# cscott/compressjs

Measured on AMD Instinct MI355X. Metric: bzip2 -9 compress MB/s on enwik8-shaped input, higher is better.
Workload: dtype u8; 1 GPU; synthetic enwik8-shaped text with phrase reuse calibrated to enwik8's bzip2 -9 ratio (compressjs_amd.synth.enwik_like, seed 2025), 100000000 bytes per GPU, bzip2 -9, 899981-byte blocks; BASELINE.json configs[2]; input_bytes=100000000, compressed_bytes=29488912, blocks_in_flight=128

## Files before the change

compressjs_amd/csrc/devutil.h:

```cpp
#pragma once
#include "cjs_common.h"

extern "C" __device__ int cjs_writelane(int val, int lane, int old) __asm("llvm.amdgcn.writelane.i32");

__device__ __forceinline__ u64 bitset1_b64(u64 m, u32 b) {
#if defined(__AMDGCN__)
    asm("s_bitset1_b64 %0, %1" : "+s"(m) : "s"(b));
    return m;
#else
    return m | (1ull << (b & 63u));
#endif
}

__device__ __forceinline__ u64 bitset0_b64(u64 m, u32 b) {
#if defined(__AMDGCN__)
    asm("s_bitset0_b64 %0, %1" : "+s"(m) : "s"(b));
    return m;
#else
    return m & ~(1ull << (b & 63u));
#endif
}

__device__ __forceinline__ u32 be_sel(u32 sh) {
#if defined(__AMDGCN__)
// ... 20 lines not shown
#if defined(__AMDGCN__)
    asm volatile("s_waitcnt lgkmcnt(0)\n\ts_barrier" ::: "memory");
#else
    __syncthreads();
#endif
}

__device__ __forceinline__ u64 match_any(u32 d, int nbits, bool valid) {
    u64 m = __ballot(valid);
    for (int i = 0; i < nbits; i++) {
        const bool bit = (d >> i) & 1u;
        const u64 b = __ballot(bit);
        m &= bit ? b : ~b;
    }
    return m;
}

__device__ __forceinline__ u32 block_excl_scan_256(u32 v, u32* sh) {
    const u32 tid = threadIdx.x;
    if (tid < 256) sh[tid] = v;
    __syncthreads();
    for (u32 off = 1; off < 256; off <<= 1) {
        u32 t = 0;
        if (tid < 256 && tid >= off) t = sh[tid - off];
        __syncthreads();
        if (tid < 256) sh[tid] += t;
        __syncthreads();
    }
    const u32 incl = tid < 256 ? sh[tid] : 0;
    __syncthreads();
    return incl - v;
}


__device__ __forceinline__ u32 wave_incl_scan_u32(u32 v) {
    const u32 lane = threadIdx.x & 63u;
    for (u32 off = 1; off < 64; off <<= 1) {
        const u32 u = __shfl_up(v, off);
        if (lane >= off) v += u;
    }
    return v;
}

__device__ __forceinline__ u32 wave_incl_scan_dpp(u32 v) {
    v += (u32)__builtin_amdgcn_update_dpp(0, (int)v, 0x111, 0xf, 0xf, true);
    v += (u32)__builtin_amdgcn_update_dpp(0, (int)v, 0x112, 0xf, 0xf, true);
    v += (u32)__builtin_amdgcn_update_dpp(0, (int)v, 0x114, 0xf, 0xf, true);
    v += (u32)__builtin_amdgcn_update_dpp(0, (int)v, 0x118, 0xf, 0xf, true);
    v += (u32)__builtin_amdgcn_update_dpp(0, (int)v, 0x142, 0xa, 0xf, false);
    v += (u32)__builtin_amdgcn_update_dpp(0, (int)v, 0x143, 0xc, 0xf, false);
    return v;
}
__device__ __forceinline__ u32 wave_sum_dpp(u32 v) { return (u32)__builtin_amdgcn_readlane((int)wave_incl_scan_dpp(v), 63); }

__device__ __forceinline__ u32 block_excl_scan_1024(u32 v, u32* sh, u32* total) {
    const u32 tid = threadIdx.x, w = tid >> 6, lane = tid & 63u;
    const u32 nw = (blockDim.x + 63u) >> 6;
    const u32 incl = wave_incl_scan_u32(v);
    if (lane == 63u) sh[w] = incl;
    __syncthreads();
    if (w == 0) {
        const u32 t = lane < nw ? sh[lane] : 0u;
        const u32 ti = wave_incl_scan_u32(t);
        if (lane < nw) sh[lane] = ti - t;
        if (lane == 63u) sh[17] = ti;
    }
    __syncthreads();
    const u32 r = sh[w] + incl - v;
    *total = sh[17];
    __syncthreads();
    return r;
}


__device__ __forceinline__ bool xcd_block_tile(u32 nb, u32& b, u32& t) {
    const u32 T = gridDim.x;
    const u32 L = blockIdx.x + T * blockIdx.y;
    const u32 xcd = L & 7u, r = L >> 3;
    t = r % T;
    b = xcd + 8u * (r / T);
    return b < nb;
}
```

compressjs_amd/csrc/k0_plan.h:

```cpp
#pragma once
#include "pipeline.h"
#include "devutil.h"

#define K0_TILE 4096
#define K0_NONE 0ull

__device__ __forceinline__ u32 k0_g(u64 k) {
    const u64 q = k / 255u;
    const u32 r = (u32)(k - q * 255u);
    return (u32)(5u * q) + (r < 4u ? r : 5u);
}
__device__ __forceinline__ u32 k0_c(u64 k) {
    const u32 sub = (u32)(k % 255u);
    return sub < 3u ? 1u : (sub == 3u ? 2u : 0u);
}

__device__ __forceinline__ void load16(const K0Buf& K, u64 j0, u8* b) {
    if (j0 + 16u <= K.in_len && ((((uintptr_t)K.in) + j0) & 15u) == 0) {
        const uint4 v = *(const uint4*)(K.in + j0);
        const u32 w[4] = {v.x, v.y, v.z, v.w};
#pragma unroll
        for (int k = 0; k < 16; k++) b[k] = (u8)(w[k >> 2] >> (8 * (k & 3)));
    } else {
#pragma unroll
        for (int k = 0; k < 16; k++) b[k] = j0 + k < K.in_len ? K.in[j0 + k] : 0;
    }
}

__device__ __forceinline__ u64 tile_runstarts(const K0Buf& K, u64 t, u64 rs_in, u8* b, u64* sh, u32& hm) {
    const u32 tid = threadIdx.x;
    const u64 j0 = t * K0_TILE + tid * 16u;
    u8 prev = 0;
    if (j0 > 0 && j0 - 1 < K.in_len) prev = K.in[j0 - 1];
    load16(K, j0, b);
    const u32 nv = j0 >= K.in_len ? 0u : (K.in_len - j0 < 16u ? (u32)(K.in_len - j0) : 16u);
    u32 heads = (j0 == 0 || b[0] != prev) ? 1u : 0u;
#pragma unroll
    for (int k = 1; k < 16; k++) heads |= b[k] != b[k - 1] ? 1u << k : 0u;
    heads &= (1u << nv) - 1u;
    hm = heads;
    u32 v = heads ? tid * 16u + 32u - (u32)__clz((int)heads) : 0u;
    const u32 lane = tid & 63u, w = tid >> 6;
    u32* sh32 = (u32*)sh;
    for (u32 off = 1; off < 64; off <<= 1) {
        const u32 u = (u32)__shfl_up((int)v, off);
        if (lane >= off && u > v) v = u;
    }
    if (lane == 63u) sh32[w] = v;
    __syncthreads();
    u32 before = (u32)__shfl_up((int)v, 1u);
    if (lane == 0) before = 0;
    for (u32 ww = 0; ww < w; ww++) if (sh32[ww] > before) before = sh32[ww];
    __syncthreads();
    return before ? t * K0_TILE + before - 1u : rs_in;
}
__device__ __forceinline__ u64 tile_runstarts(const K0Buf& K, u64 t, u64 rs_in, u8* b, u64* sh) {
    u32 hm;
    return tile_runstarts(K, t, rs_in, b, sh, hm);
}
__device__ __forceinline__ u32 k0_mod255(u64 d) { return (d >> 32) ? (u32)(d % 255u) : (u32)d % 255u; }

static __device__ u64 k0_evalC(const K0Buf& K, u64 i, u64* sh, u32* sh32) {
    if (i >= K.in_len) return K.tileC[K.ntiles];
// ... 126 lines not shown
```

compressjs_amd/csrc/k0_rle1.hip:

```cpp
#include "pipeline.h"
#include "crc_dev.h"
#include "devutil.h"
#include "k0_plan.h"

#define K0_TPW 4u
__global__ __launch_bounds__(256) void k0_tile_last(K0Buf K) {
    const u32 tid = threadIdx.x, lane = tid & 63u, w = tid >> 6;
    __shared__ u64 wl[K0_TPW][4];
    u8 b[K0_TPW][16];
    u8 prev[K0_TPW];
#pragma unroll
    for (u32 q = 0; q < K0_TPW; q++) {
        const u64 j0 = ((u64)blockIdx.x * K0_TPW + q) * K0_TILE + tid * 16u;
        prev[q] = 0;
        if (j0 < K.in_len) {
            load16(K, j0, b[q]);
            if (j0) prev[q] = K.in[j0 - 1];
        }
    }
#pragma unroll
    for (u32 q = 0; q < K0_TPW; q++) {
        const u64 j0 = ((u64)blockIdx.x * K0_TPW + q) * K0_TILE + tid * 16u;
        u64 mine = K0_NONE;
        if (j0 < K.in_len) {
#pragma unroll
            for (int k = 0; k < 16; k++) {
                const u64 j = j0 + k;
                if (j < K.in_len && (j == 0 || b[q][k] != (k ? b[q][k - 1] : prev[q]))) mine = j + 1;
            }
        }
        const u64 has = __ballot(mine != K0_NONE);
        const u64 top = __shfl(mine, has ? 63 - __clzll((long long)has) : 0);
        if (lane == 0) wl[q][w] = has ? top : K0_NONE;
    }
    __syncthreads();
    if (tid < K0_TPW) {
        const u64 t = (u64)blockIdx.x * K0_TPW + tid;
        if (t < K.ntiles) {
            u64 last = K0_NONE;
            for (u32 ww = 0; ww < 4u; ww++) if (wl[tid][ww] != K0_NONE) last = wl[tid][ww];
            K.tileA[t] = last;
            K.tileB[t] = last;
        }
    }
}

template <bool MAX>
__device__ __forceinline__ u64 scan_op(u64 a, u64 b) { return MAX ? (a > b ? a : b) : a + b; }

template <bool MAX>
__global__ __launch_bounds__(256) void k0_scan_local(u64* data, u64* chunkTot, u64 n) {
    __shared__ u64 sh[256];
    const u64 c0 = (u64)blockIdx.x * 1024u;
    const u32 tid = threadIdx.x;
    u64 v[4], run = 0;
    for (int k = 0; k < 4; k++) {
        const u64 i = c0 + tid * 4u + k;
        v[k] = i < n ? data[i] : 0;
    }
    u64 tot = 0;
    for (int k = 0; k < 4; k++) tot = scan_op<MAX>(tot, v[k]);
    sh[tid] = tot;
    __syncthreads();
    for (u32 off = 1; off < 256; off <<= 1) {
        u64 tv = 0;
        if (tid >= off) tv = sh[tid - off];
        __syncthreads();
        if (tid >= off) sh[tid] = scan_op<MAX>(sh[tid], tv);
        __syncthreads();
    }
    run = tid ? sh[tid - 1] : 0;
    for (int k = 0; k < 4; k++) {
        const u64 i = c0 + tid * 4u + k;
        if (i < n) data[i] = run;
        run = scan_op<MAX>(run, v[k]);
    }
    if (tid == 255) chunkTot[blockIdx.x] = sh[255];
}

template <bool MAX>
__global__ __launch_bounds__(1024) void k0_scan_chunks(u64* chunkTot, u64 nchunks, u64* total, u64* reset) {
    __shared__ u64 sh[1024];
    __shared__ u64 carry;
    const u32 tid = threadIdx.x;
    if (tid == 0) carry = 0;
    __syncthreads();
    for (u64 c0 = 0; c0 < nchunks; c0 += 1024) {
        const u64 i = c0 + tid;
        const u64 v = i < nchunks ? chunkTot[i] : 0;
        sh[tid] = v;
        __syncthreads();
        for (u32 off = 1; off < 1024; off <<= 1) {
            u64 tv = 0;
            if (tid >= off) tv = sh[tid - off];
            __syncthreads();
            if (tid >= off) sh[tid] = scan_op<MAX>(sh[tid], tv);
            __syncthreads();
        }
        const u64 ex = scan_op<MAX>(carry, tid ? sh[tid - 1] : 0);
        if (i < nchunks) chunkTot[i] = ex;
        __syncthreads();
        if (tid == 1023) carry = scan_op<MAX>(carry, sh[1023]);
        __syncthreads();
    }
    if (tid == 0 && total) *total = carry;
    if (tid == 0 && reset) *reset = ~0ull;
}

template <bool MAX>
__global__ __launch_bounds__(256) void k0_scan_apply(u64* data, const u64* chunkTot, u64 n) {
    const u64 c0 = (u64)blockIdx.x * 1024u;
    const u64 base = chunkTot[blockIdx.x];
    for (int k = 0; k < 4; k++) {
        const u64 i = c0 + (u64)k * 256u + threadIdx.x;
        if (i < n) data[i] = scan_op<MAX>(base, data[i]);
    }
}

__global__ __launch_bounds__(256) void k0_tile_cost(K0Buf K) {
    const u64 t = blockIdx.x;
    __shared__ u64 sh[256];
    __shared__ u32 tot;
    if (threadIdx.x == 0) tot = 0;
    u8 b[16];
    const u64 rsin_raw = K.tileA[t];
    const u64 rs_in = rsin_raw != K0_NONE ? rsin_raw - 1 : 0;
    u32 hm;
    const u64 rs = tile_runstarts(K, t, rs_in, b, sh, hm);
    const u64 j0 = t * K0_TILE + threadIdx.x * 16u;
    const u32 nv = j0 >= K.in_len ? 0u : (K.in_len - j0 < 16u ? (u32)(K.in_len - j0) : 16u);
    u32 c = 0, sub = 0;
    if (nv) {
        sub = (hm & 1u) ? 0u : k0_mod255(j0 - rs);
        c = sub < 3u ? 1u : (sub == 3u ? 2u : 0u);
#pragma unroll
        for (u32 k = 1; k < 16; k++) {
            sub = ((hm >> k) & 1u) ? 0u : (sub == 254u ? 0u : sub + 1u);
            c += k < nv ? (sub < 3u ? 1u : (sub == 3u ? 2u : 0u)) : 0u;
        }
    }
    const u32 wsum = wave_incl_scan_dpp(c);
    if ((threadIdx.x & 63u) == 63u) atomicAdd(&tot, wsum);
    __syncthreads();
    if (threadIdx.x == 0) K.tileC[t] = tot;
}

__global__ __launch_bounds__(256) void k0_chain_spec(K0Buf K, u32 cap) {
    __shared__ u64 sh[256];
    __shared__ u32 sh32[4];
    const u64 total = K.tileC[K.ntiles];
    const u64 nfull = total / cap;
    const u64 j = (u64)blockIdx.x + 1;
    if (j > nfull) return;
    u64 ce = 0;
    const u64 e = k0_searchC(K, j * (u64)cap, 0, sh, sh32, &ce);
    if (threadIdx.x == 0) {
        bool bad = e > K.in_len || ce != j * (u64)cap;
        if (!bad && e < K.in_len && e > 0 && K.in[e - 1] == K.in[e]) {
            const u8 c = K.in[e];
            u32 len = 2;
            for (u64 q = e + 1; q < K.in_len && len < 4 && K.in[q] == c; q++) len++;
            for (u64 q = e - 1; q > 0 && len < 4 && K.in[q - 1] == c; q--) len++;
            bad = len >= 4;
        }
        K.specEnd[j] = e;
        K.specC[j] = ce;
        if (bad) atomicMin((unsigned long long*)K.specBad, (unsigned long long)j);
    }
}

__global__ __launch_bounds__(256) void k0_chain(K0Buf K, u32 cap) {
    __shared__ u64 sh[256];
    __shared__ u32 sh32[4];
    const u64 total = K.tileC[K.ntiles];
    const u64 nfull = total / cap;
    u64 kb0 = *K.specBad < nfull ? *K.specBad : nfull;
    if (kb0 > K.maxBlocks) kb0 = K.maxBlocks;
    for (u64 k = threadIdx.x; k < kb0; k += 256u) {
        const u64 s0 = k ? K.specEnd[k] : 0;
        K.blkStart[k] = s0;
        K.blkEnd[k] = K.specEnd[k + 1];
        K.blkN[k] = cap;
        K.blkAdj[k] = k * (u64)cap;
        K.blkRe[k] = s0;
    }
    u64 s = kb0 ? K.specEnd[kb0] : 0, cnext = kb0 ? K.specC[kb0] : 0;
    bool have_cnext = true;
    u32 kb = (u32)kb0;
    while (s < K.in_len && kb < K.maxBlocks) {
        const bool cut = s > 0 && K.in[s - 1] == K.in[s];
        u64 e = s, adj = 0, re = s;
        u32 n = 0;
        bool done = false;
        u64 pre = 0, cbase = 0;
        if (cut) {
            re = k0_run_end(K, s, sh);
            const u64 L = re - s;
// ... 142 lines not shown
__global__ __launch_bounds__(1024) void k0_crc(K0Buf K, Pipe P, u32 first_block) {
    const u32 b = blockIdx.y, kb = first_block + b;
    if (kb >= *K.nBlocks) return;
    const u64 s = K.blkStart[kb], e = K.blkEnd[kb];
    const u32 parts = gridDim.x;
    __shared__ u32 tab[CRC_TAB_WORDS];
    __shared__ u32 pw[40];
    __shared__ u32 acc;
    const u64 part = (((e - s + parts - 1u) / parts) + 15u) & ~(u64)15;
    const u64 ps = s + blockIdx.x * part < e ? s + blockIdx.x * part : e;
    const u64 pe = ps + part < e ? ps + part : e;
    if (ps >= pe) return;
    const u32 c = crc_range_raw(K.in, ps, pe, e, tab, pw, &acc);
    if (threadIdx.x == 0) atomicXor(&P.crc[b], c);
}

size_t k0_bytes(u64 in_len, u32 cap) {
    const u64 ntiles = (in_len + K0_TILE - 1) / K0_TILE;
    const u64 nchunks = (ntiles + 1 + 1023) / 1024;
    const u64 maxBlocks = in_len / (cap / 2 + 1) + 2;
    size_t tot = 0;
    tot += 3 * (((ntiles + 2) * 8 + 255) & ~(size_t)255);
    tot += ((nchunks + 1) * 8 + 255) & ~(size_t)255;
    tot += 6 * (((maxBlocks + 2) * 8 + 255) & ~(size_t)255) + ((maxBlocks * 4 + 255) & ~(size_t)255) + 512;
    return tot;
}

void k0_carve(K0Buf& K, const u8* d_in, u64 in_len, u32 cap, void* ws) {
    K.in = d_in;
    K.in_len = in_len;
    K.ntiles = (in_len + K0_TILE - 1) / K0_TILE;
    K.nchunks = (K.ntiles + 1 + 1023) / 1024;
    K.maxBlocks = (u32)(in_len / (cap / 2 + 1) + 2);
    char* p = (char*)ws;
    const size_t ta = ((K.ntiles + 2) * 8 + 255) & ~(size_t)255;
    K.tileA = (u64*)p; p += ta;
    K.tileB = (u64*)p; p += ta;
    K.tileC = (u64*)p; p += ta;
    K.chunk = (u64*)p; p += ((K.nchunks + 1) * 8 + 255) & ~(size_t)255;
    const size_t bb = ((size_t)K.maxBlocks * 8 + 255) & ~(size_t)255;
    K.blkStart = (u64*)p; p += bb;
    K.blkEnd = (u64*)p; p += bb;
    K.blkAdj = (u64*)p; p += bb;
    K.blkRe = (u64*)p; p += bb;
    K.blkN = (u32*)p; p += ((size_t)K.maxBlocks * 4 + 255) & ~(size_t)255;
    const size_t sb = (((size_t)K.maxBlocks + 2) * 8 + 255) & ~(size_t)255;
    K.specEnd = (u64*)p; p += sb;
    K.specC = (u64*)p; p += sb;
    K.nBlocks = (u32*)p; p += 256;
    K.specBad = (u64*)p;
}

int k0_scans(K0Buf K, hipStream_t stream) {
    const u32 nt = (u32)K.ntiles, nc = (u32)K.nchunks;
    hipLaunchKernelGGL(k0_tile_last, dim3((nt + K0_TPW - 1u) / K0_TPW), dim3(256), 0, stream, K);
    hipLaunchKernelGGL(k0_scan_local<true>, dim3(nc), dim3(256), 0, stream, K.tileA, K.chunk, K.ntiles);
    hipLaunchKernelGGL(k0_scan_chunks<true>, dim3(1), dim3(1024), 0, stream, K.chunk, K.nchunks, (u64*)nullptr, (u64*)nullptr);
    hipLaunchKernelGGL(k0_scan_apply<true>, dim3(nc), dim3(256), 0, stream, K.tileA, (const u64*)K.chunk, K.ntiles);
    hipLaunchKernelGGL(k0_tile_cost, dim3(nt), dim3(256), 0, stream, K);
    hipLaunchKernelGGL(k0_scan_local<false>, dim3(nc), dim3(256), 0, stream, K.tileC, K.chunk, K.ntiles);
    hipLaunchKernelGGL(k0_scan_chunks<false>, dim3(1), dim3(1024), 0, stream, K.chunk, K.nchunks, K.tileC + K.ntiles, K.specBad);
    hipLaunchKernelGGL(k0_scan_apply<false>, dim3(nc), dim3(256), 0, stream, K.tileC, (const u64*)K.chunk, K.ntiles);
    HIP_CHECK_RET(hipGetLastError());
    return CJS_OK;
}

int k0_prepass(K0Buf K, u32 cap, hipStream_t stream) {
    if (K.in_len == 0) {
        HIP_CHECK_RET(hipMemsetAsync(K.nBlocks, 0, 4, stream));
        return CJS_OK;
    }
    const int rc = k0_scans(K, stream);
    if (rc) return rc;
    const u32 nspec = (u32)(K.in_len * 5 / 4 / cap + 2 < K.maxBlocks ? K.in_len * 5 / 4 / cap + 2 : K.maxBlocks);
    hipLaunchKernelGGL(k0_chain_spec, dim3(nspec), dim3(256), 0, stream, K, cap);
    hipLaunchKernelGGL(k0_chain, dim3(1), dim3(256), 0, stream, K, cap);
    HIP_CHECK_RET(hipGetLastError());
    return CJS_OK;
}

__global__ __launch_bounds__(256) void k0_phase_spec(K0Buf K, u32 cap, u64 t0) {
    __shared__ u64 sh[256];
    __shared__ u32 sh32[4];
    const u64 total = K.tileC[K.ntiles];
    const u64 m = blockIdx.x;
    const u64 t = t0 + m * (u64)cap;
    if (t > total) { if (threadIdx.x == 0) { K.specEnd[m] = K.in_len + 1; K.specC[m] = 0; } return; }
    u64 ce = 0, e = 0;
    if (t) e = k0_searchC(K, t, 0, sh, sh32, &ce);
    if (threadIdx.x == 0) {
        bool bad = e > K.in_len || ce != t;
        if (!bad && e < K.in_len && e > 0 && K.in[e - 1] == K.in[e]) {
            const u8 c = K.in[e];
            u32 len = 2;
            for (u64 q = e + 1; q < K.in_len && len < 4 && K.in[q] == c; q++) len++;
            for (u64 q = e - 1; q > 0 && len < 4 && K.in[q - 1] == c; q--) len++;
            bad = len >= 4;
        }
        K.specEnd[m] = e;
        K.specC[m] = ce;
        if (bad) atomicMin((unsigned long long*)K.specBad, (unsigned long long)m);
    }
}

__global__ __launch_bounds__(256) void k0_phase_chain(K0Buf K, u32 cap, u64 t0, u64 own_len, u32 last, u32 nbound) {
    __shared__ u64 sh[256];
    __shared__ u32 sh32[4];
    __shared__ u32 nb, fail, stop;
    const u32 tid = threadIdx.x;
    if (tid == 0) { nb = 0; fail = 0; stop = nbound; }
    __syncthreads();
    const u64 total = K.tileC[K.ntiles];
    const u64 badraw = *K.specBad;
    const u32 bad = badraw < (u64)nbound ? (u32)badraw : nbound;
    for (u32 m = tid; m < nbound; m += 256u) {
// ... 113 lines not shown
```

compressjs_amd/csrc/k5_pack.hip:

```cpp
#include "pipeline.h"

__device__ __forceinline__ u32 bswap32(u32 v) {
    return (v >> 24) | ((v >> 8) & 0xFF00u) | ((v << 8) & 0xFF0000u) | (v << 24);
}

__device__ __forceinline__ void put_bits_lds(u32* words, u32 pos, u32 nbits, u32 value) {
    if (nbits == 0) return;
    const u32 wi = pos >> 5, sh = pos & 31u;
    const u64 v = ((u64)value << (64u - nbits)) >> sh;
    atomicOr(&words[wi], (u32)(v >> 32));
    const u32 lo = (u32)v;
    if (lo) atomicOr(&words[wi + 1], lo);
}

__device__ __forceinline__ u32 mtf6_index(u32 list, u32 s) {
    u32 j = 0;
    while (((list >> (4u * j)) & 15u) != s) j++;
    return j;
}
__device__ __forceinline__ u32 mtf6_front(u32 list, u32 j, u32 s) {
    const u32 lowmask = (1u << (4u * j)) - 1u;
    const u32 keep = list & ~((lowmask << 4) | 15u);
    return keep | ((list & lowmask) << 4) | s;
}

#define K5_MAX_SEL 18432
__global__ __launch_bounds__(256) void k5_header(Pipe P) {
    const u32 b = blockIdx.x;
    const u32 n = P.nlen[b];
    const u32 tid = threadIdx.x;
    if (n == 0) { if (tid == 0) P.hbits[b] = 0; return; }
    __shared__ u32 hw[K5_HDR_WORDS];
    __shared__ u32 sh[256];
    __shared__ int lastT[6][256];
    __shared__ u32 s_cursor;
    for (u32 i = tid; i < K5_HDR_WORDS; i += 256) hw[i] = 0;
    __syncthreads();
    const u32 alpha = P.alpha[b], G = P.ngroups[b], nSel = P.nsel[b];
    const int S = (int)alpha + 2;
    __shared__ __attribute__((aligned(16))) u8 sel[K5_MAX_SEL];
    {
        const u8* gsel = P.sel + (size_t)b * P.selPitch;
        const u32 nw4 = ((nSel < K5_MAX_SEL ? nSel : K5_MAX_SEL) + 3u) >> 2;
        for (u32 i = tid; i < nw4; i += 256) ((u32*)sel)[i] = ((const u32*)gsel)[i];
    }
    if (tid == 0) {
        put_bits_lds(hw, 0, 24, 0x314159u);
        put_bits_lds(hw, 24, 24, 0x265359u);
        put_bits_lds(hw, 48, 32, P.crc[b]);
        put_bits_lds(hw, 80, 1, 0);
        put_bits_lds(hw, 81, 24, P.pidx[b]);
        const u32* used8 = P.used + (size_t)b * 8;
        u32 cur = 105, map = 0;
        for (int i = 0; i < 16; i++) {
            const u32 r = (used8[i >> 1] >> ((i & 1) * 16)) & 0xFFFFu;
            if (r) map |= 1u << (15 - i);
        }
        put_bits_lds(hw, cur, 16, map);
        cur += 16;
        for (int i = 0; i < 16; i++) {
            const u32 r = (used8[i >> 1] >> ((i & 1) * 16)) & 0xFFFFu;
            if (r) {
                u32 rev = 0;
                for (int j = 0; j < 16; j++) if (r & (1u << j)) rev |= 1u << (15 - j);
                put_bits_lds(hw, cur, 16, rev);
                cur += 16;
            }
        }
        put_bits_lds(hw, cur, 3, G);
        put_bits_lds(hw, cur + 3, 15, nSel);
        s_cursor = cur + 18;
    }
    __syncthreads();
    u32 cursor = s_cursor;
    if (alpha >= G) {
        const u32 chunk = (nSel + 255u) / 256u;
        const u32 lo = tid * chunk < nSel ? tid * chunk : nSel;
        const u32 hi = lo + chunk < nSel ? lo + chunk : nSel;
        int lastp[6];
#pragma unroll
        for (int t = 0; t < 6; t++) lastp[t] = K5_NONE;
        for (u32 i = lo; i < hi; i++) {
            const u32 s = sel[i];
#pragma unroll
            for (int t = 0; t < 6; t++) if (s == (u32)t) lastp[t] = (int)i;
        }
#pragma unroll
        for (int t = 0; t < 6; t++) lastT[t][tid] = lastp[t];
        __syncthreads();
        if (tid < 6) {
            int cur = -1 - (int)tid;
            for (int k = 0; k < 256; k++) {
                const int v = lastT[tid][k];
                lastT[tid][k] = cur;
                cur = cur > v ? cur : v;
            }
        }
        __syncthreads();
        u32 list = 0;
        {
            int Ls[6];
#pragma unroll
            for (int t = 0; t < 6; t++) Ls[t] = lastT[t][tid];
#pragma unroll
            for (int t = 0; t < 6; t++) {
                u32 r = 0;
#pragma unroll
                for (int u = 0; u < 6; u++) r += (Ls[u] > Ls[t]) ? 1u : 0u;
                list |= (u32)t << (4u * r);
            }
        }
        const u32 list0 = list;
        u32 bits = 0;
        for (u32 i = lo; i < hi; i++) {
            const u32 s = sel[i];
            const u32 j = mtf6_index(list, s);
            list = mtf6_front(list, j, s);
            bits += j + 1u;
        }
        u32 off = cursor + block_excl_scan_256(bits, sh);
        list = list0;
        for (u32 i = lo; i < hi; i++) {
            const u32 s = sel[i];
            const u32 j = mtf6_index(list, s);
            list = mtf6_front(list, j, s);
            put_bits_lds(hw, off, j + 1u, ((1u << j) - 1u) << 1);
            off += j + 1u;
        }
        __syncthreads();
        if (tid == 255) s_cursor = off;
        __syncthreads();
        cursor = s_cursor;
    } else {
        if (tid == 0) {
            int M[6];
            const int mlen = (int)alpha;
            for (int i = 0; i < mlen; i++) M[i] = i;
            u32 off = cursor;
            for (u32 i = 0; i < nSel; i++) {
                const int s = sel[i];
                int j;
                for (j = 0; j < (int)G; j++) if (j < mlen && M[j] == s) break;
                const int src = j < mlen ? M[j] : 0;
                for (int k = j; k > 0; k--) if (k < mlen) M[k] = M[k - 1];
                if (mlen > 0) M[0] = src;
                put_bits_lds(hw, off, (u32)j + 1u, ((1u << j) - 1u) << 1);
                off += (u32)j + 1u;
            }
            s_cursor = off;
        }
        __syncthreads();
        cursor = s_cursor;
    }
    for (u32 t = 0; t < G; t++) {
        const u8* lens = P.lens + ((size_t)b * CJS_MAX_GROUPS + t) * CJS_LEN_PITCH;
        if (tid == 0) put_bits_lds(hw, cursor, 5, lens[0]);
        u32 nb0 = 0, nb1 = 0;
        const int i0 = 2 * (int)tid, i1 = i0 + 1;
        int l0 = 0, lp0 = 0, l1 = 0;
        if (i0 < S) { l0 = lens[i0]; lp0 = i0 ? lens[i0 - 1] : l0; nb0 = 2u * (u32)(l0 > lp0 ? l0 - lp0 : lp0 - l0) + 1u; }
        if (i1 < S) { l1 = lens[i1]; nb1 = 2u * (u32)(l1 > l0 ? l1 - l0 : l0 - l1) + 1u; }
        u32 off = cursor + 5u + block_excl_scan_256(nb0 + nb1, sh);
        if (i0 < S) {
            const u32 val = lp0 < l0 ? 2u : 3u;
            for (u32 d = 0; d + 1u < nb0; d += 2u) put_bits_lds(hw, off + d, 2, val);
            off += nb0;
        }
        if (i1 < S) {
            const u32 val = l0 < l1 ? 2u : 3u;
            for (u32 d = 0; d + 1u < nb1; d += 2u) put_bits_lds(hw, off + d, 2, val);
            off += nb1;
        }
        __syncthreads();
        if (tid == 255) s_cursor = off;
        __syncthreads();
        cursor = s_cursor;
    }
    const u32 nw = (cursor + 31u) >> 5;
    u32* out = P.hdr + (size_t)b * K5_HDR_WORDS;
    for (u32 i = tid; i < nw; i += 256) out[i] = hw[i];
    if (tid == 0) P.hbits[b] = cursor;
}

__global__ __launch_bounds__(256) void k5_tilescan(Pipe P) {
    const BatchGeom g = P.g;
    const u32 b = blockIdx.x, tid = threadIdx.x;
    __shared__ u32 sh[256];
    __shared__ u32 carry;
    const u32 nSel = P.nlen[b] ? P.nsel[b] : 0u;
    if (tid == 0) carry = P.nlen[b] ? P.hbits[b] : 0u;
    __syncthreads();
    const u16* cost = P.selCost + (size_t)b * P.selPitch;
    u32* cnt = P.tileBits + (size_t)b * K5_TILES(g);
    for (u32 t0 = 0; t0 < K5_TILES(g); t0 += 256) {
        const u32 t = t0 + tid;
        u32 v = 0;
        const u32 g0 = t * K5_TGROUPS;
        if (g0 + K5_TGROUPS <= nSel) {
            const uint4* c4 = (const uint4*)(cost + g0);
#pragma unroll
            for (u32 k = 0; k < K5_TGROUPS / 8u; k++) {
                const uint4 q = c4[k];
                v += (q.x & 0xFFFFu) + (q.x >> 16) + (q.y & 0xFFFFu) + (q.y >> 16) + (q.z & 0xFFFFu) + (q.z >> 16) + (q.w & 0xFFFFu) + (q.w >> 16);
            }
        } else for (u32 gi = g0; gi < nSel; gi++) v += cost[gi];
        const u32 ex = block_excl_scan_256(v, sh);
        const u32 base = carry;
        if (t < K5_TILES(g)) cnt[t] = base + ex;
        __syncthreads();
        if (tid == 255) carry = base + ex + v;
        __syncthreads();
    }
    if (tid == 0) P.bitlen[b] = carry;
}

__global__ __launch_bounds__(64) void k5_blockscan(Pipe P) {
    if (threadIdx.x != 0) return;
    u64 bits = P.ss->bits;
    u32 crc = P.ss->crc;
    for (u32 b = 0; b < P.g.nb; b++) {
        P.bitoff[b] = bits;
        if (P.nlen[b]) {
            bits += P.bitlen[b];
            crc = ((crc << 1) | (crc >> 31)) ^ P.crc[b];
        }
    }
    if (((bits + 80u + 7u) >> 3) + 8u > P.outCapBytes) P.ss->overflow = 1;
    P.ss->bits = bits;
    P.ss->crc = crc;
    if (P.snap) *P.snap = bits;
}

#define K5_STAGE_WORDS ((K5_TILE * 20u + 62u) / 32u + 2u)
__device__ __forceinline__ void or_word(u32* out, u64 wi, u32 word) {
    if (word) atomicOr(&out[wi], bswap32(word));
}

__global__ __launch_bounds__(256) void k5_pack(Pipe P) {
    const BatchGeom g = P.g;
    const u32 b = blockIdx.y, t = blockIdx.x;
    if (P.nlen[b] == 0 || P.ss->overflow) return;
    const u32 pos = P.pos[b];
    const u32 t0 = t * K5_TILE;
    const u32 tid = threadIdx.x;
    const u64 boff = P.bitoff[b];
    if (t == 0) {
        const u32 hb = P.hbits[b];
        const u32 nw = (hb + 31u) >> 5;
        const u32* hdr = P.hdr + (size_t)b * K5_HDR_WORDS;
        const u32 s = (u32)(boff & 31u);
        const u64 w0 = boff >> 5;
        for (u32 k = tid; k <= nw; k += 256) {
            const u32 cur = k < nw ? hdr[k] : 0u;
            const u32 prev = k > 0 ? hdr[k - 1] : 0u;
            const u32 v = s ? ((prev << (32u - s)) | (cur >> s)) : cur;
            or_word(P.out, w0 + k, v);
        }
    }
    if (t0 >= pos) return;
    __shared__ u32 codes[CJS_MAX_GROUPS][CJS_LEN_PITCH];
    __shared__ u32 sh[256];
    __shared__ u32 stage[K5_STAGE_WORDS];
    __shared__ u32 s_tot;
    const u32 G = P.ngroups[b];
// ... 48 lines not shown
            }
        }
        if (nacc) atomicOr(&stage[wi], (u32)(acc << (32u - nacc)));
    }
    __syncthreads();
    for (u32 j = tid; j < nw; j += 256) {
        const u32 v = stage[j];
        if (j == 0u || j + 1u == nw) or_word(P.out, w0 + j, v);
        else P.out[w0 + j] = bswap32(v);
    }
}

__global__ void k5_begin(Pipe P, int level) {
    if (threadIdx.x == 0 && blockIdx.x == 0) {
        if (level > 0) P.out[0] = bswap32(0x425A6800u | (u32)('0' + level));
        P.ss->bits = level > 0 ? 32 : 0;
        P.ss->crc = 0;
        P.ss->overflow = 0;
    }
}
__global__ void k5_end(Pipe P) {
    if (threadIdx.x != 0 || blockIdx.x != 0 || P.ss->overflow) return;
    const u64 pos = P.ss->bits;
    const u32 parts[3] = {0x177245u, 0x385090u, P.ss->crc};
    const u32 nb[3] = {24, 24, 32};
    u64 p = pos;
    for (int k = 0; k < 3; k++) {
        const u32 sh = (u32)(p & 31u);
        const u64 v = ((u64)parts[k] << (64u - nb[k])) >> sh;
        or_word(P.out, p >> 5, (u32)(v >> 32));
        or_word(P.out, (p >> 5) + 1, (u32)v);
        p += nb[k];
    }
    P.ss->bits = p;
}

int k5_stream_begin(Pipe P, int level, hipStream_t stream, bool zero) {
    if (zero) HIP_CHECK_RET(hipMemsetAsync(P.out, 0, P.outCapBytes, stream));
    hipLaunchKernelGGL(k5_begin, dim3(1), dim3(64), 0, stream, P, level);
    HIP_CHECK_RET(hipGetLastError());
    return CJS_OK;
}

int k5_stream_end(Pipe P, hipStream_t stream) {
    hipLaunchKernelGGL(k5_end, dim3(1), dim3(64), 0, stream, P);
    HIP_CHECK_RET(hipGetLastError());
    return CJS_OK;
}

int k5_run(Pipe P, u32 max_n, hipStream_t stream, hipEvent_t after, hipEvent_t done, hipEvent_t crc_ready, const K5Docs* docs, u32 first_block) {
    const BatchGeom g = P.g;
    const u32 tiles = (max_n + 1 + K5_TILE - 1) / K5_TILE;
    if (crc_ready) HIP_CHECK_RET(hipStreamWaitEvent(stream, crc_ready, 0));
    hipLaunchKernelGGL(k5_header, dim3(g.nb), dim3(256), 0, stream, P);
    hipLaunchKernelGGL(k5_tilescan, dim3(g.nb), dim3(256), 0, stream, P);
    if (after) HIP_CHECK_RET(hipStreamWaitEvent(stream, after, 0));
    if (docs) {
        const int rc = k5_docscan_run(P, *docs, first_block, stream);
        if (rc) return rc;
    } else hipLaunchKernelGGL(k5_blockscan, dim3(1), dim3(64), 0, stream, P);
    if (done) HIP_CHECK_RET(hipEventRecord(done, stream));
    hipLaunchKernelGGL(k5_pack, dim3(tiles, g.nb), dim3(256), 0, stream, P);
    HIP_CHECK_RET(hipGetLastError());
    return CJS_OK;
}

__global__ __launch_bounds__(256) void k5_shift_bits(const u8* in, u64 nbytes, u32 s, u8* out) {
    const u64 i = (u64)blockIdx.x * 256u + threadIdx.x;
    if (i > nbytes) return;
    const u32 cur = i < nbytes ? in[i] : 0u;
    const u32 prev = i ? in[i - 1] : 0u;
    out[i] = (u8)((cur >> s) | (prev << (8u - s)));
}
int k5_shift_bits_run(const u8* d_in, u64 nbytes, u32 s, u8* d_out, hipStream_t stream) {
    hipLaunchKernelGGL(k5_shift_bits, dim3((u32)((nbytes + 256) / 256)), dim3(256), 0, stream, d_in, nbytes, s & 7u, d_out);
    HIP_CHECK_RET(hipGetLastError());
    return CJS_OK;
}
```

Baseline: 15710 MB/s.

## Fuse RLE1 tile scans into two kernels and merge header with tilescan

Replaces the eight-kernel RLE1 planning sequence (tile-last, three-pass max scan, tile-cost, three-pass sum scan) with a tile summary kernel that computes last run start, leading-run length and in-tile cost in one pass, plus a single 1024-thread kernel that does both scans and fixes up the cost of the leading run algebraically. The bzip2 header kernel grows to 1024 threads, uses DPP wave scans instead of serial LDS scans, stores MTF positions so the selector MTF pass runs once, writes all code-length deltas in one scan, and absorbs the tilescan kernel. The aim is to cut launch count, serial single-thread loops and repeated input reads. The cost is a single-block scan over all tiles and more complex carry and boundary logic.

```diff
diff --git a/compressjs_amd/csrc/devutil.h b/compressjs_amd/csrc/devutil.h
--- a/compressjs_amd/csrc/devutil.h
+++ b/compressjs_amd/csrc/devutil.h
@@ -96,6 +96,18 @@
     return v;
 }
 __device__ __forceinline__ u32 wave_sum_dpp(u32 v) { return (u32)__builtin_amdgcn_readlane((int)wave_incl_scan_dpp(v), 63); }
+template <bool MAX>
+__device__ __forceinline__ u32 wave_incl_scan_dpp_op(u32 v) {
+#define CJS_DPP_STEP(ctrl, rows, bc) { const u32 u = (u32)__builtin_amdgcn_update_dpp(0, (int)v, ctrl, rows, 0xf, bc); v = MAX ? (u > v ? u : v) : v + u; }
+    CJS_DPP_STEP(0x111, 0xf, true)
+    CJS_DPP_STEP(0x112, 0xf, true)
+    CJS_DPP_STEP(0x114, 0xf, true)
+    CJS_DPP_STEP(0x118, 0xf, true)
+    CJS_DPP_STEP(0x142, 0xa, false)
+    CJS_DPP_STEP(0x143, 0xc, false)
+#undef CJS_DPP_STEP
+    return v;
+}
 
 __device__ __forceinline__ u32 block_excl_scan_1024(u32 v, u32* sh, u32* total) {
     const u32 tid = threadIdx.x, w = tid >> 6, lane = tid & 63u;
diff --git a/compressjs_amd/csrc/k0_plan.h b/compressjs_amd/csrc/k0_plan.h
--- a/compressjs_amd/csrc/k0_plan.h
+++ b/compressjs_amd/csrc/k0_plan.h
@@ -9,6 +9,10 @@
     const u64 q = k / 255u;
     const u32 r = (u32)(k - q * 255u);
     return (u32)(5u * q) + (r < 4u ? r : 5u);
+}
+__device__ __forceinline__ u32 k0_g32(u32 k) {
+    const u32 q = k / 255u, r = k - q * 255u;
+    return 5u * q + (r < 4u ? r : 5u);
 }
 __device__ __forceinline__ u32 k0_c(u64 k) {
     const u32 sub = (u32)(k % 255u);
diff --git a/compressjs_amd/csrc/k0_rle1.hip b/compressjs_amd/csrc/k0_rle1.hip
--- a/compressjs_amd/csrc/k0_rle1.hip
+++ b/compressjs_amd/csrc/k0_rle1.hip
@@ -4,9 +4,11 @@
 #include "k0_plan.h"
 
 #define K0_TPW 4u
-__global__ __launch_bounds__(256) void k0_tile_last(K0Buf K) {
+__device__ __forceinline__ u32 k0_cost_of(u32 sub) { return sub < 3u ? 1u : (sub == 3u ? 2u : 0u); }
+
+__global__ __launch_bounds__(256) void k0_tile_summary(K0Buf K) {
     const u32 tid = threadIdx.x, lane = tid & 63u, w = tid >> 6;
-    __shared__ u64 wl[K0_TPW][4];
+    __shared__ u32 wlast[K0_TPW][4], wfirst[K0_TPW][4], wcost[K0_TPW][4];
     u8 b[K0_TPW][16];
     u8 prev[K0_TPW];
 #pragma unroll
@@ -18,131 +20,143 @@
             if (j0) prev[q] = K.in[j0 - 1];
         }
     }
+    u32 hm[K0_TPW], vm[K0_TPW], nvs[K0_TPW];
 #pragma unroll
     for (u32 q = 0; q < K0_TPW; q++) {
         const u64 j0 = ((u64)blockIdx.x * K0_TPW + q) * K0_TILE + tid * 16u;
-        u64 mine = K0_NONE;
-        if (j0 < K.in_len) {
-#pragma unroll
-            for (int k = 0; k < 16; k++) {
-                const u64 j = j0 + k;
-                if (j < K.in_len && (j == 0 || b[q][k] != (k ? b[q][k - 1] : prev[q]))) mine = j + 1;
-            }
-        }
-        const u64 has = __ballot(mine != K0_NONE);
-        const u64 top = __shfl(mine, has ? 63 - __clzll((long long)has) : 0);
-        if (lane == 0) wl[q][w] = has ? top : K0_NONE;
+        const u32 nv = j0 >= K.in_len ? 0u : (K.in_len - j0 < 16u ? (u32)(K.in_len - j0) : 16u);
+        u32 heads = 0;
+        if (nv) {
+            heads = (j0 == 0 || b[q][0] != prev[q]) ? 1u : 0u;
+#pragma unroll
+            for (int k = 1; k < 16; k++) heads |= b[q][k] != b[q][k - 1] ? 1u << k : 0u;
+            heads &= (1u << nv) - 1u;
+        }
+        hm[q] = heads;
+        nvs[q] = nv;
+        const u32 v = wave_incl_scan_dpp_op<true>(heads ? tid * 16u + 32u - (u32)__clz((int)heads) : 0u);
+        vm[q] = v;
+        const u64 has = __ballot(heads != 0u);
+        const u32 fh = (u32)__shfl((int)heads, has ? __ffsll((long long)has) - 1 : 0);
+        if (lane == 63u) wlast[q][w] = v;
+        if (lane == 0) wfirst[q][w] = has ? (w * 64u + (u32)__ffsll((long long)has) - 1u) * 16u + (u32)__ffs((int)fh) : 0u;
+    }
+    __syncthreads();
+#pragma unroll
+    for (u32 q = 0; q < K0_TPW; q++) {
+        u32 before = (u32)__builtin_amdgcn_update_dpp(0, (int)vm[q], 0x138, 0xf, 0xf, false);
+        for (u32 ww = 0; ww < w; ww++) if (wlast[q][ww] > before) before = wlast[q][ww];
+        const u32 heads = hm[q], nv = nvs[q];
+        u32 c = 0;
+        if (nv) {
+            bool in = (heads & 1u) || before;
+            u32 sub = (heads & 1u) || !before ? 0u : (tid * 16u + 1u - before) % 255u;
+            c = in ? k0_cost_of(sub) : 0u;
+#pragma unroll
+            for (u32 k = 1; k < 16; k++) {
+                const bool h = (heads >> k) & 1u;
+                in = in || h;
+                sub = h ? 0u : (sub == 254u ? 0u : sub + 1u);
+                c += (k < nv && in) ? k0_cost_of(sub) : 0u;
+            }
+        }
+        const u32 wsum = wave_incl_scan_dpp(c);
+        if (lane == 63u) wcost[q][w] = wsum;
     }
     __syncthreads();
     if (tid < K0_TPW) {
         const u64 t = (u64)blockIdx.x * K0_TPW + tid;
         if (t < K.ntiles) {
-            u64 last = K0_NONE;
-            for (u32 ww = 0; ww < 4u; ww++) if (wl[tid][ww] != K0_NONE) last = wl[tid][ww];
-            K.tileA[t] = last;
-            K.tileB[t] = last;
-        }
-    }
-}
-
+            u32 last = 0, first = 0, cost = 0;
+            for (u32 ww = 0; ww < 4u; ww++) {
+                if (wlast[tid][ww] > last) last = wlast[tid][ww];
+                if (!first) first = wfirst[tid][ww];
+                cost += wcost[tid][ww];
+            }
+            const u64 left = K.in_len - t * K0_TILE;
+            const u32 lead = first ? first - 1u : (left < K0_TILE ? (u32)left : (u32)K0_TILE);
+            K.tileB[t] = last ? t * K0_TILE + last : K0_NONE;
+            K.tileC[t] = (u64)lead << 32 | cost;
+        }
+    }
+}
+
+#define K0_SROWS 8u
 template <bool MAX>
-__device__ __forceinline__ u64 scan_op(u64 a, u64 b) { return MAX ? (a > b ? a : b) : a + b; }
-
-template <bool MAX>
-__global__ __launch_bounds__(256) void k0_scan_local(u64* data, u64* chunkTot, u64 n) {
-    __shared__ u64 sh[256];
-    const u64 c0 = (u64)blockIdx.x * 1024u;
-    const u32 tid = threadIdx.x;
-    u64 v[4], run = 0;
-    for (int k = 0; k < 4; k++) {
-        const u64 i = c0 + tid * 4u + k;
-        v[k] = i < n ? data[i] : 0;
-    }
-    u64 tot = 0;
-    for (int k = 0; k < 4; k++) tot = scan_op<MAX>(tot, v[k]);
-    sh[tid] = tot;
-    __syncthreads();
-    for (u32 off = 1; off < 256; off <<= 1) {
-        u64 tv = 0;
-        if (tid >= off) tv = sh[tid - off];
+__device__ __forceinline__ void k0_scan_wave_totals(u32* wt) {
+    const u32 lane = threadIdx.x & 63u;
+    const u32 a = wt[2u * lane], b = wt[2u * lane + 1u];
+    const u32 inc = wave_incl_scan_dpp_op<MAX>(MAX ? (a > b ? a : b) : a + b);
+    const u32 ex = (u32)__builtin_amdgcn_update_dpp(0, (int)inc, 0x138, 0xf, 0xf, false);
+    wt[2u * lane] = ex;
+    wt[2u * lane + 1u] = MAX ? (a > ex ? a : ex) : a + ex;
+    if (lane == 63u) wt[16u * K0_SROWS] = inc;
+}
+static_assert(16u * K0_SROWS == 128u, "k0_scan_wave_totals: two wave totals per lane of wave 0");
+
+__global__ __launch_bounds__(1024) void k0_tile_scan(K0Buf K) {
+    __shared__ u32 wtM[16u * K0_SROWS + 1u], wtC[16u * K0_SROWS + 1u];
+    const u32 tid = threadIdx.x, lane = tid & 63u, w = tid >> 6;
+    u32 carryM = 0;
+    u64 carryC = 0;
+    for (u64 base = 0; base < K.ntiles; base += K0_SROWS * 1024u) {
+        u32 m[K0_SROWS];
+        u64 pc[K0_SROWS];
+#pragma unroll
+        for (u32 r = 0; r < K0_SROWS; r++) {
+            const u64 i = base + r * 1024u + tid;
+            m[r] = (i > 0 && i < K.ntiles && K.tileB[i - 1] != K0_NONE) ? (u32)i : 0u;
+            pc[r] = i < K.ntiles ? K.tileC[i] : 0ull;
+        }
+#pragma unroll
+        for (u32 r = 0; r < K0_SROWS; r++) {
+            m[r] = wave_incl_scan_dpp_op<true>(m[r]);
+            if (lane == 63u) wtM[r * 16u + w] = m[r];
+        }
         __syncthreads();
-        if (tid >= off) sh[tid] = scan_op<MAX>(sh[tid], tv);
+        if (w == 0) k0_scan_wave_totals<true>(wtM);
         __syncthreads();
-    }
-    run = tid ? sh[tid - 1] : 0;
-    for (int k = 0; k < 4; k++) {
-        const u64 i = c0 + tid * 4u + k;
-        if (i < n) data[i] = run;
-        run = scan_op<MAX>(run, v[k]);
-    }
-    if (tid == 255) chunkTot[blockIdx.x] = sh[255];
-}
-
-template <bool MAX>
-__global__ __launch_bounds__(1024) void k0_scan_chunks(u64* chunkTot, u64 nchunks, u64* total, u64* reset) {
-    __shared__ u64 sh[1024];
-    __shared__ u64 carry;
-    const u32 tid = threadIdx.x;
-    if (tid == 0) carry = 0;
-    __syncthreads();
-    for (u64 c0 = 0; c0 < nchunks; c0 += 1024) {
-        const u64 i = c0 + tid;
-        const u64 v = i < nchunks ? chunkTot[i] : 0;
-        sh[tid] = v;
+        u32 c[K0_SROWS];
+        u64 a[K0_SROWS];
+#pragma unroll
+        for (u32 r = 0; r < K0_SROWS; r++) {
+            const u64 i = base + r * 1024u + tid;
+            const u32 o = wtM[r * 16u + w];
+            if (o > m[r]) m[r] = o;
+            if (carryM > m[r]) m[r] = carryM;
+            a[r] = (i < K.ntiles && m[r]) ? K.tileB[m[r] - 1u] : K0_NONE;
+        }
+        if (wtM[16u * K0_SROWS] > carryM) carryM = wtM[16u * K0_SROWS];
+#pragma unroll
+        for (u32 r = 0; r < K0_SROWS; r++) {
+            const u64 i = base + r * 1024u + tid;
+            const u32 lead = (u32)(pc[r] >> 32);
+            c[r] = (u32)pc[r];
+            if (i < K.ntiles) {
+                K.tileA[i] = a[r];
+                if (lead) {
+                    const u64 d = i * K0_TILE - (a[r] != K0_NONE ? a[r] - 1 : 0);
+                    c[r] += ((d + lead) >> 32) ? k0_g(d + lead) - k0_g(d) : k0_g32((u32)d + lead) - k0_g32((u32)d);
+                }
+            }
+            pc[r] = c[r];
+            c[r] = wave_incl_scan_dpp_op<false>(c[r]);
+            if (lane == 63u) wtC[r * 16u + w] = c[r];
+        }
         __syncthreads();
-        for (u32 off = 1; off < 1024; off <<= 1) {
-            u64 tv = 0;
-            if (tid >= off) tv = sh[tid - off];
-            __syncthreads();
-            if (tid >= off) sh[tid] = scan_op<MAX>(sh[tid], tv);
-            __syncthreads();
-        }
-        const u64 ex = scan_op<MAX>(carry, tid ? sh[tid - 1] : 0);
-        if (i < nchunks) chunkTot[i] = ex;
+        if (w == 0) k0_scan_wave_totals<false>(wtC);
         __syncthreads();
-        if (tid == 1023) carry = scan_op<MAX>(carry, sh[1023]);
-        __syncthreads();
-    }
-    if (tid == 0 && total) *total = carry;
-    if (tid == 0 && reset) *reset = ~0ull;
-}
-
-template <bool MAX>
-__global__ __launch_bounds__(256) void k0_scan_apply(u64* data, const u64* chunkTot, u64 n) {
-    const u64 c0 = (u64)blockIdx.x * 1024u;
-    const u64 base = chunkTot[blockIdx.x];
-    for (int k = 0; k < 4; k++) {
-        const u64 i = c0 + (u64)k * 256u + threadIdx.x;
-        if (i < n) data[i] = scan_op<MAX>(base, data[i]);
-    }
-}
-
-__global__ __launch_bounds__(256) void k0_tile_cost(K0Buf K) {
-    const u64 t = blockIdx.x;
-    __shared__ u64 sh[256];
-    __shared__ u32 tot;
-    if (threadIdx.x == 0) tot = 0;
-    u8 b[16];
-    const u64 rsin_raw = K.tileA[t];
-    const u64 rs_in = rsin_raw != K0_NONE ? rsin_raw - 1 : 0;
-    u32 hm;
-    const u64 rs = tile_runstarts(K, t, rs_in, b, sh, hm);
-    const u64 j0 = t * K0_TILE + threadIdx.x * 16u;
-    const u32 nv = j0 >= K.in_len ? 0u : (K.in_len - j0 < 16u ? (u32)(K.in_len - j0) : 16u);
-    u32 c = 0, sub = 0;
-    if (nv) {
-        sub = (hm & 1u) ? 0u : k0_mod255(j0 - rs);
-        c = sub < 3u ? 1u : (sub == 3u ? 2u : 0u);
-#pragma unroll
-        for (u32 k = 1; k < 16; k++) {
-            sub = ((hm >> k) & 1u) ? 0u : (sub == 254u ? 0u : sub + 1u);
-            c += k < nv ? (sub < 3u ? 1u : (sub == 3u ? 2u : 0u)) : 0u;
-        }
-    }
-    const u32 wsum = wave_incl_scan_dpp(c);
-    if ((threadIdx.x & 63u) == 63u) atomicAdd(&tot, wsum);
-    __syncthreads();
-    if (threadIdx.x == 0) K.tileC[t] = tot;
+#pragma unroll
+        for (u32 r = 0; r < K0_SROWS; r++) {
+            const u64 i = base + r * 1024u + tid;
+            if (i < K.ntiles) K.tileC[i] = carryC + wtC[r * 16u + w] + (c[r] - (u32)pc[r]);
+        }
+        carryC += wtC[16u * K0_SROWS];
+    }
+    if (tid == 0) {
+        K.tileC[K.ntiles] = carryC;
+        *K.specBad = ~0ull;
+    }
 }
 
 __global__ __launch_bounds__(256) void k0_chain_spec(K0Buf K, u32 cap) {
@@ -391,15 +405,9 @@
 }
 
 int k0_scans(K0Buf K, hipStream_t stream) {
-    const u32 nt = (u32)K.ntiles, nc = (u32)K.nchunks;
-    hipLaunchKernelGGL(k0_tile_last, dim3((nt + K0_TPW - 1u) / K0_TPW), dim3(256), 0, stream, K);
-    hipLaunchKernelGGL(k0_scan_local<true>, dim3(nc), dim3(256), 0, stream, K.tileA, K.chunk, K.ntiles);
-    hipLaunchKernelGGL(k0_scan_chunks<true>, dim3(1), dim3(1024), 0, stream, K.chunk, K.nchunks, (u64*)nullptr, (u64*)nullptr);
-    hipLaunchKernelGGL(k0_scan_apply<true>, dim3(nc), dim3(256), 0, stream, K.tileA, (const u64*)K.chunk, K.ntiles);
-    hipLaunchKernelGGL(k0_tile_cost, dim3(nt), dim3(256), 0, stream, K);
-    hipLaunchKernelGGL(k0_scan_local<false>, dim3(nc), dim3(256), 0, stream, K.tileC, K.chunk, K.ntiles);
-    hipLaunchKernelGGL(k0_scan_chunks<false>, dim3(1), dim3(1024), 0, stream, K.chunk, K.nchunks, K.tileC + K.ntiles, K.specBad);
-    hipLaunchKernelGGL(k0_scan_apply<false>, dim3(nc), dim3(256), 0, stream, K.tileC, (const u64*)K.chunk, K.ntiles);
+    const u32 nt = (u32)K.ntiles;
+    hipLaunchKernelGGL(k0_tile_summary, dim3((nt + K0_TPW - 1u) / K0_TPW), dim3(256), 0, stream, K);
+    hipLaunchKernelGGL(k0_tile_scan, dim3(1), dim3(1024), 0, stream, K);
     HIP_CHECK_RET(hipGetLastError());
     return CJS_OK;
 }
diff --git a/compressjs_amd/csrc/k5_pack.hip b/compressjs_amd/csrc/k5_pack.hip
--- a/compressjs_amd/csrc/k5_pack.hip
+++ b/compressjs_amd/csrc/k5_pack.hip
@@ -25,24 +25,41 @@
 }
 
 #define K5_MAX_SEL 18432
-__global__ __launch_bounds__(256) void k5_header(Pipe P) {
+#define K5_HT 1024u
+static_assert((K5_MAX_SEL + K5_HT - 1u) / K5_HT * 3u <= 64u, "k5_header keeps a thread's MTF positions, three bits each, in one u64");
+
+__device__ __forceinline__ void put_delta_lds(u32* words, u32 pos, u32 nbits, bool up) {
+    const u32 pat = up ? 0xAAAAAAAAu : 0xFFFFFFFFu;
+    if (nbits > 32u) {
+        put_bits_lds(words, pos, 32, pat);
+        put_bits_lds(words, pos + 32u, nbits - 32u, pat >> (64u - nbits));
+    } else if (nbits) put_bits_lds(words, pos, nbits, pat >> (32u - nbits));
+}
+
+__global__ __launch_bounds__(K5_HT) void k5_header(Pipe P) {
+    const BatchGeom g = P.g;
     const u32 b = blockIdx.x;
     const u32 n = P.nlen[b];
-    const u32 tid = threadIdx.x;
-    if (n == 0) { if (tid == 0) P.hbits[b] = 0; return; }
+    const u32 tid = threadIdx.x, lane = tid & 63u, w = tid >> 6;
+    u32* cnt = P.tileBits + (size_t)b * K5_TILES(g);
+    if (n == 0) {
+        for (u32 t = tid; t < K5_TILES(g); t += K5_HT) cnt[t] = 0;
+        if (tid == 0) { P.hbits[b] = 0; P.bitlen[b] = 0; }
+        return;
+    }
     __shared__ u32 hw[K5_HDR_WORDS];
-    __shared__ u32 sh[256];
-    __shared__ int lastT[6][256];
+    __shared__ u32 sh[20];
+    __shared__ u32 wmax[8][16];
     __shared__ u32 s_cursor;
-    for (u32 i = tid; i < K5_HDR_WORDS; i += 256) hw[i] = 0;
+    for (u32 i = tid; i < K5_HDR_WORDS; i += K5_HT) hw[i] = 0;
     __syncthreads();
     const u32 alpha = P.alpha[b], G = P.ngroups[b], nSel = P.nsel[b];
-    const int S = (int)alpha + 2;
+    const u32 S = alpha + 2u;
     __shared__ __attribute__((aligned(16))) u8 sel[K5_MAX_SEL];
     {
         const u8* gsel = P.sel + (size_t)b * P.selPitch;
         const u32 nw4 = ((nSel < K5_MAX_SEL ? nSel : K5_MAX_SEL) + 3u) >> 2;
-        for (u32 i = tid; i < nw4; i += 256) ((u32*)sel)[i] = ((const u32*)gsel)[i];
+        for (u32 i = tid; i < nw4; i += K5_HT) ((u32*)sel)[i] = ((const u32*)gsel)[i];
     }
     if (tid == 0) {
         put_bits_lds(hw, 0, 24, 0x314159u);
@@ -61,9 +78,7 @@
         for (int i = 0; i < 16; i++) {
             const u32 r = (used8[i >> 1] >> ((i & 1) * 16)) & 0xFFFFu;
             if (r) {
-                u32 rev = 0;
-                for (int j = 0; j < 16; j++) if (r & (1u << j)) rev |= 1u << (15 - j);
-                put_bits_lds(hw, cur, 16, rev);
+                put_bits_lds(hw, cur, 16, __brev(r) >> 16);
                 cur += 16;
             }
         }
@@ -74,34 +89,42 @@
     __syncthreads();
     u32 cursor = s_cursor;
     if (alpha >= G) {
-        const u32 chunk = (nSel + 255u) / 256u;
+        const u32 chunk = (nSel + K5_HT - 1u) / K5_HT;
         const u32 lo = tid * chunk < nSel ? tid * chunk : nSel;
         const u32 hi = lo + chunk < nSel ? lo + chunk : nSel;
-        int lastp[6];
-#pragma unroll
-        for (int t = 0; t < 6; t++) lastp[t] = K5_NONE;
+        u32 last[6];
+#pragma unroll
+        for (int t = 0; t < 6; t++) last[t] = 0;
         for (u32 i = lo; i < hi; i++) {
             const u32 s = sel[i];
 #pragma unroll
-            for (int t = 0; t < 6; t++) if (s == (u32)t) lastp[t] = (int)i;
-        }
-#pragma unroll
-        for (int t = 0; t < 6; t++) lastT[t][tid] = lastp[t];
+            for (int t = 0; t < 6; t++) if (s == (u32)t) last[t] = i + 7u;
+        }
+#pragma unroll
+        for (int t = 0; t < 6; t++) {
+            last[t] = wave_incl_scan_dpp_op<true>(last[t]);
+            if (lane == 63u) wmax[t][w] = last[t];
+        }
         __syncthreads();
-        if (tid < 6) {
-            int cur = -1 - (int)tid;
-            for (int k = 0; k < 256; k++) {
-                const int v = lastT[tid][k];
-                lastT[tid][k] = cur;
-                cur = cur > v ? cur : v;
-            }
+        if (tid < 128u) {
+            u32 v = tid < 96u ? wmax[tid >> 4][tid & 15u] : 0u, u;
+            u = (u32)__builtin_amdgcn_update_dpp(0, (int)v, 0x111, 0xf, 0xf, true); v = u > v ? u : v;
+            u = (u32)__builtin_amdgcn_update_dpp(0, (int)v, 0x112, 0xf, 0xf, true); v = u > v ? u : v;
+            u = (u32)__builtin_amdgcn_update_dpp(0, (int)v, 0x114, 0xf, 0xf, true); v = u > v ? u : v;
+            u = (u32)__builtin_amdgcn_update_dpp(0, (int)v, 0x118, 0xf, 0xf, true); v = u > v ? u : v;
+            wmax[tid >> 4][tid & 15u] = (u32)__builtin_amdgcn_update_dpp(0, (int)v, 0x111, 0xf, 0xf, true);
         }
         __syncthreads();
         u32 list = 0;
         {
-            int Ls[6];
-#pragma unroll
-            for (int t = 0; t < 6; t++) Ls[t] = lastT[t][tid];
+            u32 Ls[6];
+#pragma unroll
+            for (int t = 0; t < 6; t++) {
+                const u32 inwave = (u32)__builtin_amdgcn_update_dpp(0, (int)last[t], 0x138, 0xf, 0xf, false);
+                const u32 front = wmax[t][w];
+                Ls[t] = inwave > front ? inwave : front;
+                if (Ls[t] < 6u - (u32)t) Ls[t] = 6u - (u32)t;
+            }
 #pragma unroll
             for (int t = 0; t < 6; t++) {
                 u32 r = 0;
@@ -110,27 +133,23 @@
                 list |= (u32)t << (4u * r);
             }
         }
-        const u32 list0 = list;
         u32 bits = 0;
-        for (u32 i = lo; i < hi; i++) {
+        u64 js = 0;
+        for (u32 i = lo, k = 0; i < hi; i++, k += 3u) {
             const u32 s = sel[i];
             const u32 j = mtf6_index(list, s);
             list = mtf6_front(list, j, s);
+            js |= (u64)j << k;
             bits += j + 1u;
         }
-        u32 off = cursor + block_excl_scan_256(bits, sh);
-        list = list0;
-        for (u32 i = lo; i < hi; i++) {
-            const u32 s = sel[i];
-            const u32 j = mtf6_index(list, s);
-            list = mtf6_front(list, j, s);
+        u32 tot;
+        u32 off = cursor + block_excl_scan_1024(bits, sh, &tot);
+        for (u32 i = lo; i < hi; i++, js >>= 3) {
+            const u32 j = (u32)js & 7u;
             put_bits_lds(hw, off, j + 1u, ((1u << j) - 1u) << 1);
             off += j + 1u;
         }
-        __syncthreads();
-        if (tid == 255) s_cursor = off;
-        __syncthreads();
-        cursor = s_cursor;
+        cursor += tot;
     } else {
         if (tid == 0) {
             int M[6];
@@ -152,47 +171,40 @@
         __syncthreads();
         cursor = s_cursor;
     }
-    for (u32 t = 0; t < G; t++) {
-        const u8* lens = P.lens + ((size_t)b * CJS_MAX_GROUPS + t) * CJS_LEN_PITCH;
-        if (tid == 0) put_bits_lds(hw, cursor, 5, lens[0]);
-        u32 nb0 = 0, nb1 = 0;
-        const int i0 = 2 * (int)tid, i1 = i0 + 1;
-        int l0 = 0, lp0 = 0, l1 = 0;
-        if (i0 < S) { l0 = lens[i0]; lp0 = i0 ? lens[i0 - 1] : l0; nb0 = 2u * (u32)(l0 > lp0 ? l0 - lp0 : lp0 - l0) + 1u; }
-        if (i1 < S) { l1 = lens[i1]; nb1 = 2u * (u32)(l1 > l0 ? l1 - l0 : l0 - l1) + 1u; }
-        u32 off = cursor + 5u + block_excl_scan_256(nb0 + nb1, sh);
-        if (i0 < S) {
-            const u32 val = lp0 < l0 ? 2u : 3u;
-            for (u32 d = 0; d + 1u < nb0; d += 2u) put_bits_lds(hw, off + d, 2, val);
-            off += nb0;
-        }
-        if (i1 < S) {
-            const u32 val = l0 < l1 ? 2u : 3u;
-            for (u32 d = 0; d + 1u < nb1; d += 2u) put_bits_lds(hw, off + d, 2, val);
-            off += nb1;
-        }
-        __syncthreads();
-        if (tid == 255) s_cursor = off;
-        __syncthreads();
-        cursor = s_cursor;
-    }
+    {
+        u32 l[2], lp[2], nb[2];
+#pragma unroll
+        for (u32 q = 0; q < 2u; q++) {
+            const u32 p = 2u * tid + q;
+            l[q] = lp[q] = nb[q] = 0;
+            if (p < G * S) {
+                const u32 t = p / S, i = p - t * S;
+                const u8* lens = P.lens + ((size_t)b * CJS_MAX_GROUPS + t) * CJS_LEN_PITCH;
+                l[q] = lens[i];
+                lp[q] = i ? lens[i - 1u] : l[q];
+                nb[q] = 2u * (l[q] > lp[q] ? l[q] - lp[q] : lp[q] - l[q]) + 1u + (i ? 0u : 0x100u + 5u);
+            }
+        }
+        u32 tot;
+        u32 off = cursor + block_excl_scan_1024((nb[0] & 0xFFu) + (nb[1] & 0xFFu), sh, &tot);
+#pragma unroll
+        for (u32 q = 0; q < 2u; q++) {
+            if (nb[q] & 0x100u) { put_bits_lds(hw, off, 5, l[q]); off += 5u; nb[q] -= 0x105u; }
+            if (nb[q]) {
+                put_delta_lds(hw, off, nb[q] - 1u, lp[q] < l[q]);
+                off += nb[q];
+            }
+        }
+        cursor += tot;
+    }
+    __syncthreads();
     const u32 nw = (cursor + 31u) >> 5;
     u32* out = P.hdr + (size_t)b * K5_HDR_WORDS;
-    for (u32 i = tid; i < nw; i += 256) out[i] = hw[i];
+    for (u32 i = tid; i < nw; i += K5_HT) out[i] = hw[i];
     if (tid == 0) P.hbits[b] = cursor;
-}
-
-__global__ __launch_bounds__(256) void k5_tilescan(Pipe P) {
-    const BatchGeom g = P.g;
-    const u32 b = blockIdx.x, tid = threadIdx.x;
-    __shared__ u32 sh[256];
-    __shared__ u32 carry;
-    const u32 nSel = P.nlen[b] ? P.nsel[b] : 0u;
-    if (tid == 0) carry = P.nlen[b] ? P.hbits[b] : 0u;
-    __syncthreads();
     const u16* cost = P.selCost + (size_t)b * P.selPitch;
-    u32* cnt = P.tileBits + (size_t)b * K5_TILES(g);
-    for (u32 t0 = 0; t0 < K5_TILES(g); t0 += 256) {
+    u32 carry = cursor;
+    for (u32 t0 = 0; t0 < K5_TILES(g); t0 += K5_HT) {
         const u32 t = t0 + tid;
         u32 v = 0;
         const u32 g0 = t * K5_TGROUPS;
@@ -204,12 +216,10 @@
                 v += (q.x & 0xFFFFu) + (q.x >> 16) + (q.y & 0xFFFFu) + (q.y >> 16) + (q.z & 0xFFFFu) + (q.z >> 16) + (q.w & 0xFFFFu) + (q.w >> 16);
             }
         } else for (u32 gi = g0; gi < nSel; gi++) v += cost[gi];
-        const u32 ex = block_excl_scan_256(v, sh);
-        const u32 base = carry;
-        if (t < K5_TILES(g)) cnt[t] = base + ex;
-        __syncthreads();
-        if (tid == 255) carry = base + ex + v;
-        __syncthreads();
+        u32 tot;
+        const u32 ex = block_excl_scan_1024(v, sh, &tot);
+        if (t < K5_TILES(g)) cnt[t] = carry + ex;
+        carry += tot;
     }
     if (tid == 0) P.bitlen[b] = carry;
 }
@@ -364,8 +374,7 @@
     const BatchGeom g = P.g;
     const u32 tiles = (max_n + 1 + K5_TILE - 1) / K5_TILE;
     if (crc_ready) HIP_CHECK_RET(hipStreamWaitEvent(stream, crc_ready, 0));
-    hipLaunchKernelGGL(k5_header, dim3(g.nb), dim3(256), 0, stream, P);
-    hipLaunchKernelGGL(k5_tilescan, dim3(g.nb), dim3(256), 0, stream, P);
+    hipLaunchKernelGGL(k5_header, dim3(g.nb), dim3(K5_HT), 0, stream, P);
     if (after) HIP_CHECK_RET(hipStreamWaitEvent(stream, after, 0));
     if (docs) {
         const int rc = k5_docscan_run(P, *docs, first_block, stream);
```

New measurement: 15790 MB/s, median of 6. Within noise of the previous version (+0.6%).
